# PaulMullowney/hypre

Hardware: AMD Instinct MI355X
Metric: BoomerAMG V-cycle DOF/s (256^3 7-pt Laplacian per GPU, l1-Jacobi V(1,1), fp64) (higher is better)
Workload: dtype f64; 1 GPU; 256x256x256 7-pt Laplacian, 1 rank(s) 1x1x1, PMIS + ext+i(4) + l1-Jacobi V(1,1); transport=none, replicated_from_level=-1, coarse_tail_graph_from_level=-1, coarse_tail_graph_nodes=0, one_workgroup_tail_from_level=6, levels=9

## Files before the change

### hypre_amd/binding.py

```python
import ctypes as C
import os

import numpy as np

HERE = os.path.dirname(os.path.abspath(__file__))
LIB_PATH = os.environ.get("HYPRE_AMD_LIB") or os.path.join(HERE, "lib", "libhypre_amd.so")

HYPRE_MEMORY_HOST = 0
HYPRE_MEMORY_DEVICE = 1

Int = C.c_int
BigInt = C.c_longlong
Real = C.c_double
IntP = C.POINTER(C.c_int)
BigIntP = C.POINTER(C.c_longlong)
RealP = C.POINTER(C.c_double)


class HypreAmdError(RuntimeError):
    pass


class CSRMatrix(C.Structure):
    _fields_ = [("i", IntP), ("j", IntP), ("big_j", BigIntP), ("num_rows", Int), ("num_cols", Int),
# ... 153 lines not shown
    "hypre_CSRMatrixMatvecT": (Int, [Real, CSRp, Vecp, Real, Vecp]),
    "hypre_CSRMatrixMatvecDevice": (Int, [Int, Real, CSRp, Vecp, Real, Vecp, Vecp, Int]),
    "hypre_CSRMatrixSpMVDevice": (Int, [Int, Real, CSRp, Vecp, Real, Vecp, Int]),
    "hypre_amd_CSRMatrixInvalidatePlan": (Int, [CSRp]),
    "hypre_amd_CSRMatrixVerifyPlan": (Int, [CSRp]),
    "hypre_amd_CSRMatrixSetImmutable": (Int, [CSRp, Int]),
    "hypre_amd_CSRMatrixPlanForm": (Int, [CSRp]),
    "hypre_amd_PlanTestFailAlloc": (Int, [Int, Int]),
    "hypre_amd_SetMixedPrecisionValues": (Int, [Int]),
    "hypre_amd_SpmvSetRowSlices": (Int, [Int]),
    "hypre_amd_SpmvSetFusedMultivectors": (Int, [Int]),
    "hypre_amd_SpmvFusedMultivectorLaunches": (Int, []),
    "hypre_amd_CSRMatrixPlanRowSlices": (Int, [CSRp, IntP, IntP]),
    "hypre_amd_CSRMatrixSortRows": (Int, [CSRp, Int]),
    "hypre_amd_SpmvSetBandPolicy": (Int, [Int, Int, Int]),
    "hypre_amd_SpmvSetVariant": (Int, [Int, Int]),
    "hypre_amd_CSRMatrixPlanInfo": (Int, [CSRp, IntP, IntP]),
    "hypre_amd_CSRMatrixPlanStaging": (Int, [CSRp, IntP, RealP]),
    "hypre_amd_SpmvSetValueCodes": (Int, [Int]),
    "hypre_amd_SpmvSetSliceForm": (Int, [Int]),
    "hypre_amd_CSRMatrixPlanSliceForm": (Int, [CSRp]),
    "hypre_amd_SpmvSetSliceClasses": (Int, [Int]),
    "hypre_amd_CSRMatrixPlanSliceClasses": (Int, [CSRp]),
    "hypre_amd_CSRMatrixPlanSliceClassHistogram": (Int, [CSRp, C.POINTER(Int), C.POINTER(Int), C.POINTER(BigInt)]),
    "hypre_amd_CSRMatrixPlanValueCodes": (Int, [CSRp]),
    "hypre_SeqVectorSetConstantValues": (Int, [Vecp, Real]),
    "hypre_SeqVectorCopy": (Int, [Vecp, Vecp]),
    "hypre_SeqVectorScale": (Int, [Real, Vecp]),
    "hypre_SeqVectorAxpy": (Int, [Real, Vecp, Vecp]),
    "hypre_SeqVectorAxpyz": (Int, [Real, Vecp, Real, Vecp, Vecp]),
    "hypre_SeqVectorInnerProd": (Real, [Vecp, Vecp]),
    "hypre_SeqVectorElmdivpy": (Int, [Vecp, Vecp, Vecp]),
    "hypre_SeqVectorElmdivpyMarked": (Int, [Vecp, Vecp, Vecp, IntP, Int]),
    "hypre_SeqVectorSetConstantValuesDevice": (Int, [Vecp, Real]),
    "hypre_SeqVectorScaleDevice": (Int, [Real, Vecp]),
    "hypre_SeqVectorAxpyDevice": (Int, [Real, Vecp, Vecp]),
    "hypre_SeqVectorAxpyzDevice": (Int, [Real, Vecp, Real, Vecp, Vecp]),
    "hypre_SeqVectorInnerProdDevice": (Real, [Vecp, Vecp]),
    "hypre_SeqVectorElmdivpyDevice": (Int, [Vecp, Vecp, Vecp, IntP, Int]),
    "hypreDevice_IVAXPY": (Int, [Int, RealP, RealP, RealP]),
    "hypreDevice_IVAXPYMarked": (Int, [Int, RealP, RealP, RealP, IntP, Int]),
    "hypreDevice_DiagScaleVector2": (Int, [Int, Int, RealP, RealP, Real, RealP, RealP, Int]),
    "hypre_ParCSRMatrixCreate": (ParCSRp, [Int, BigInt, BigInt, BigIntP, BigIntP, Int, Int, Int]),
    "hypre_ParCSRMatrixInitialize_v2": (Int, [ParCSRp, Int]),
    "hypre_ParCSRMatrixDestroy": (Int, [ParCSRp]),
    "hypre_ParCSRMatrixMigrate": (Int, [ParCSRp, Int]),
# ... 230 lines not shown
```

### hypre_amd/csrc/internal.hpp

```cpp
#pragma once

#include <hip/hip_runtime.h>
#include <cstdio>
#include <cstdlib>
#include <cstring>
#include <cstdint>
#include <vector>

#include "HYPRE_amd_utilities.h"
#include "hypre_amd_seq_mv.h"
#include "hypre_amd_comm.h"
#include "hypre_amd_parcsr_mv.h"

#define HIP_CHECK(call)                                                          \
   do {                                                                          \
      hipError_t e_ = (call);                                                    \
      if (e_ != hipSuccess) {                                                    \
         char msg_[512];                                                         \
         snprintf(msg_, sizeof(msg_), "HIP error %d (%s) in %s", (int) e_,       \
                  hipGetErrorString(e_), #call);                                 \
         hypre_error_handler(__FILE__, __LINE__, HYPRE_ERROR_GENERIC, msg_);     \
      }                                                                          \
   } while (0)

// ... 131 lines not shown
void watch_release(MatrixWatch &w);
int *take_stale_slot(int **device_view);
void give_stale_slot(int *slot);
void launch_matrix_fingerprint(const int *Ai, const int *Aj, const double *Aa, int n, int nnz, unsigned long long *fp, int *stale,
                               int record, hipStream_t s);
unsigned long long plan_generation();
bool plan_is_stale(const hypre_CSRMatrix *A);
void launch_build_fp(const HYPRE_Int *Aj, int nnz, int num_tiles, int *fp, hipStream_t s);
SpmvPlan *get_plan(hypre_CSRMatrix *A);
hypre_CSRMatrix *strict_lower_of(hypre_CSRMatrix *A);
void      drop_plan(hypre_CSRMatrix *A);
const float *fp32_values_of(hypre_CSRMatrix *A);
void      set_strict_lower(hypre_CSRMatrix *A, hypre_CSRMatrix *L);

enum SpmvOp
{
   OP_AXPBY   = 0,
   OP_JACOBI  = 1,
   OP_JACOBI_CF = 2,
   OP_TSGS    = 3,
   OP_JACOBI_MAP = 4,
   OP_AXPBY_DIV = 5,
   OP_RESID_RD = 6,
   OP_TSGS_FIRST = 7
};

struct SpmvArgs
{
   const HYPRE_Int     *Ai;
   const HYPRE_Int     *Aj;
   const HYPRE_Complex *Aa;
   const float         *Aa32;
   const unsigned char *Ac8;
   const double        *dict;
   int                  ndict;
   int                  dict_rounded;
   const HYPRE_Complex *x;
   const HYPRE_Complex *b;
   HYPRE_Complex       *y;
   HYPRE_Complex       *aux;
   const HYPRE_Complex *d;
   const HYPRE_Int     *marker;
   int                  marker_val;
   HYPRE_Complex        alpha, beta;
   HYPRE_Complex        scale2;
   int                  fill;
   int                  row_offset;
   int                  last_quad;
   int                  x_last;
   int                  reduce_w;
   int                  gather_t;
   int                  xcd_map;
   const int           *tile_perm;
   const int           *tile_fp;
   int                 *stale;
   const int           *rowmap;
   int                  variant;
   int                  use_rs;
   unsigned             rot;
   int                  nnz;
};
void spmv_default_flags(SpmvArgs &a);

void launch_spmv(const SpmvPlan *plan, const SpmvArgs &args, SpmvOp op, hipStream_t s);
bool spmv_with_scaled_quotient(hypre_CSRMatrix *M, const double *x, double *y, double w, const double *d, double *u);
bool launch_spmv_mv(const SpmvPlan *plan, const SpmvArgs &args, int nv, long xstride, long bstride, long ystride, hipStream_t s);
long &spmv_mv_launches();
bool &spmv_fused_multivectors();
void launch_spmv_rownnz(const HYPRE_Int *rownnz, int num_rownnz, const SpmvArgs &args, hipStream_t s);
void launch_spmv_allrows_update(int num_rows, const SpmvArgs &args, hipStream_t s);
bool device_value_codes(const double *Aa, size_t nnz, unsigned char **codes_out, double **dict_out, double **dict32_out, int *ndict_out,
                        hipStream_t s);
bool device_build_slice_form(SpmvPlan *p, const hypre_CSRMatrix *A, hipStream_t s);
bool device_build_row_slices(SpmvPlan *p, const hypre_CSRMatrix *A, hipStream_t s);
int  &spmv_row_slices();
bool &spmv_slice_classes();
bool &spmv_slice_form();
bool &spmv_value_codes();
void launch_build_tiles(const HYPRE_Int *Ai, int num_rows, int nnz, int num_tiles, int *d_tile_row,
                        int *d_tile_k, hipStream_t s);
void launch_build_xs(const HYPRE_Int *Aj, const int *d_tile_k, int num_tiles, int *xs_cnt, int *xs_desc, unsigned short *lidx,
                     hipStream_t s);
constexpr int SPMV_XS_SEGS = 48;
constexpr int SPMV_XS_CAP  = 4096;
int  device_max_row_nnz(const HYPRE_Int *Ai, int num_rows, hipStream_t s);
void sample_row_bands(const HYPRE_Int *Ai, const HYPRE_Int *Aj, int num_rows, int nsamples, int *host_out, hipStream_t s);

void launch_set(double *y, double v, size_t n, hipStream_t s);
// ... 95 lines not shown
```

### hypre_amd/csrc/par_solve.cpp

```cpp
#include "amg_internal.hpp"
#include <algorithm>
#include <cmath>
#include <string>

using namespace hamd;

namespace hamd {

void AmgPrivate::drop_graph()
{
   if (graph_exec) { (void) hipGraphExecDestroy(graph_exec); graph_exec = nullptr; }
   if (graph) { (void) hipGraphDestroy(graph); graph = nullptr; }
   graph_state = 0; graph_sig = 0; graph_launches = 0;
   graph_cur.clear();
}

void AmgPrivate::release_device()
{
   drop_graph();
   graph_level = -1;
   for (double *p : u_alt) { if (p) { hypre_Free(p, HYPRE_MEMORY_DEVICE); } }
   u_alt.clear(); u_alt_len.clear();
   for (double *p : diag_buf) { if (p) { hypre_Free(p, HYPRE_MEMORY_DEVICE); } }
   diag_buf.clear(); diag_len.clear();
// ... 524 lines not shown
   mix((unsigned long long) d->num_levels); mix((unsigned long long) gl);
   for (int k = 0; k < 4; k++) { mix((unsigned long long) d->grid_relax_type[k]); mix((unsigned long long) d->num_grid_sweeps[k]); }
   mix((unsigned long long) d->relax_order); mix((unsigned long long) d->cycle_type); mix((unsigned long long) d->fcycle);
   mix((unsigned long long) d->user_relax_type); mix((unsigned long long) (d->grid_relax_points != nullptr));
   mix((unsigned long long) pv->mixed_precision); mix((unsigned long long) pv->emulated_threads);
   mix((unsigned long long) (uintptr_t) d->Vtemp->local_vector->data);
   for (int l = gl; l < d->num_levels; l++)
   {
      mixd(d->relax_weight[l]); mixd(d->omega[l]);
      mix((unsigned long long) (uintptr_t) d->A_array[l]->diag->data); mix((unsigned long long) (uintptr_t) d->A_array[l]->diag->j);
      mix((unsigned long long) d->A_array[l]->diag->num_nonzeros);
      if (l < d->num_levels - 1 && d->P_array[l])
      {
         mix((unsigned long long) (uintptr_t) d->P_array[l]->diag->data);
         mix((unsigned long long) (uintptr_t) (d->P_array[l]->diagT ? d->P_array[l]->diagT->data : nullptr));
      }
      mix((unsigned long long) (uintptr_t) F[l]->local_vector->data); mix((unsigned long long) (uintptr_t) U[l]->local_vector->data);
      mix((unsigned long long) (uintptr_t) (d->l1_norms[l] ? d->l1_norms[l]->data : nullptr));
      mix((unsigned long long) (uintptr_t) (l < (int) pv->u_alt.size() ? pv->u_alt[(size_t) l] : nullptr));
      mix((unsigned long long) (uintptr_t) (l < (int) pv->diag_buf.size() ? pv->diag_buf[(size_t) l] : nullptr));
   }
   mix(plan_generation());
   mix((unsigned long long) cycle_fusion());
   mix((unsigned long long) (small_tail_on() ? pv->small_tail_nnz : 0)); mix((unsigned long long) (small_tail_forced_form() + 1));
   mix((unsigned long long) hypre_amd_SetMcLookAhead(-1));
   SpmvArgs a{};
   spmv_default_flags(a);
   mix((unsigned long long) a.variant); mix((unsigned long long) a.gather_t); mix((unsigned long long) a.xcd_map);
   return h;
}

bool is_jacobi_type(int t) { return t == 0 || t == 7 || t == 18; }
bool is_ge_type(int t) { return t == 9 || t == 19 || t == 98 || t == 99 || t == 198 || t == 199; }

}

HYPRE_Int hypre_amd_SetCycleFusion(HYPRE_Int on)
{
   if (on >= 0) { cycle_fusion() = on != 0; }
   return cycle_fusion();
}

HYPRE_Int hypre_amd_SetSmallTail(HYPRE_Int on)
{
   if (on >= 0) { small_tail_on() = on != 0; }
   return small_tail_on();
// ... 180 lines not shown
      arrived_down = false;
      int num_sweep, relax_type;
      if (L > 1) { num_sweep = d->num_grid_sweeps[cycle_param]; relax_type = d->grid_relax_type[cycle_param]; }
      else
      {
         num_sweep = d->num_grid_sweeps[0];
         relax_type = d->user_relax_type;
         if (relax_type == -1) { relax_type = 6; }
      }
      const int *cf = d->CF_marker_array[level] ? d->CF_marker_array[level]->data : nullptr;
      const double *l1 = d->l1_norms[level] ? d->l1_norms[level]->data : nullptr;
      const double *fd = F_array[level]->local_vector->data;
      LevelVec &u = lv[(size_t) level];
      const double w = d->relax_weight[level];

      const bool tail_here = pv->tail != nullptr && level == pv->tail_level;
      if (tail_here)
      {
         err = run_replicated_tail(d, pv, fd, u.home, &cycle_op_count);
         u.cur = u.home;
         zeros[(size_t) level] = 0;
         if (err) { break; }
      }
      for (int j = 0; j < ((tail_here || replayed) ? 0 : num_sweep); j++)
      {
         int relax_points = 0, relax_local = d->relax_order;
         if (L == 1 && d->max_levels > 1) { relax_points = 0; relax_local = 0; }
         else if (old_version) { relax_points = d->grid_relax_points[cycle_param][j]; }
         if (old_version && level < L - 1)
         {
            if (relax_points == 1) { cycle_op_count += A[level + 1]->d_num_nonzeros; }
            else if (relax_points == -1) { cycle_op_count += A[level]->d_num_nonzeros - A[level + 1]->d_num_nonzeros; }
         }
         else { cycle_op_count += A[level]->d_num_nonzeros; }
         if (is_ge_type(relax_type))
         {
            hypre_GaussElimSolve(d, level, relax_type);
            u.cur = u.home;
            zeros[(size_t) level] = 0;
         }
         else if (is_jacobi_type(relax_type))
         {
            int pts[2] = {relax_points, 0}, npass = 1;
            if (!old_version && relax_local == 1 && cycle_param < 3)
            {
               npass = 2;
               pts[0] = cycle_param < 2 ? 1 : -1; pts[1] = -pts[0];
            }
            const double *dg = l1;
            if (relax_type == 0 || !dg)
            {
               double *dd = pv->level_diag(level, n);
               launch_diag_first(A[level]->diag->i, A[level]->diag->data, dd, n, s);
               dg = dd;
            }
            for (int pss = 0; pss < npass; pss++)
            {
               if (zeros[(size_t) level] && relax_type != 0)
               {
                  if (presmoothed[(size_t) level]) { presmoothed[(size_t) level] = 0; }
                  else { launch_scaled_div(w, fd, dg, u.cur, pts[pss] ? cf : nullptr, pts[pss], (size_t) n, s); }
               }
               else
               {
                  dev_jacobi_sweep(A[level], fd, cf, pts[pss], w, dg, u.cur, u.other());
                  u.flip();
               }
               zeros[(size_t) level] = 0;
            }
         }
         else if (relax_type == 15)
         {
            if (j == 0)
            {
               if (pv->cg_smoothers.size() < (size_t) L) { pv->cg_smoothers.resize((size_t) L, nullptr); }
               hypre_Vector uv; hypre_ParVector up;
               wrap(&uv, u.cur, n);
               wrap_par(&up, &uv, A[level]->comm, A[level]->global_num_rows);
               up.all_zeros = zeros[(size_t) level];
               HYPRE_Solver &cg = pv->cg_smoothers[(size_t) level];
               if (!cg)
               {
                  HYPRE_ParCSRPCGCreate(A[level]->comm, &cg);
// ... 54 lines not shown
            hypre_ParVectorSetLocalSize(d->Ztemp, n);
            if (old_version) { err = hypre_BoomerAMGRelax(A[level], F_array[level], (HYPRE_Int *) cf, relax_type, relax_points, w, d->omega[level], (HYPRE_Real *) l1, &up, d->Vtemp, d->Ztemp); }
            else { err = hypre_BoomerAMGRelaxIF(A[level], F_array[level], (HYPRE_Int *) cf, relax_type, relax_local, cycle_param, w, d->omega[level], (HYPRE_Real *) l1, &up, d->Vtemp, d->Ztemp); }
            zeros[(size_t) level] = 0;
            if (hypre_error_flag) { err = 1; }
         }
         if (err) { break; }
      }
      if (err) { break; }

      if (!replayed) { --lev_counter[(size_t) level]; }
      if (!replayed && lev_counter[(size_t) level] >= 0 && level != L - 1 && !tail_here)
      {
         arrived_down = true;
         const int fine = level, coarse = level + 1;
         LevelVec &uc = lv[(size_t) coarse];
         uc.cur = uc.home;
         const int nc = A[coarse]->diag->num_rows;
         const int ctype = d->grid_relax_type[coarse == L - 1 ? 3 : 1];
         const bool overwrites_all = (is_jacobi_type(ctype) && ctype != 0 && !(d->relax_order == 1 && coarse != L - 1) &&
                                      !old_version && d->num_grid_sweeps[coarse == L - 1 ? 3 : 1] > 0) || is_ge_type(ctype);
         if (!overwrites_all) { launch_set(uc.cur, 0.0, (size_t) nc, s); }
         zeros[(size_t) coarse] = 1;
         dev_par_matvec(-1.0, A[fine], u.cur, 1.0, fd, vtemp);
         const int fuse_on = cycle_fusion();
         presmoothed[(size_t) coarse] = 0;
         bool restricted = false;
         if (fuse_on && cycle_nprocs == 1 && overwrites_all && is_jacobi_type(ctype) && d->l1_norms[coarse] && d->l1_norms[coarse]->data &&
             P[fine]->diagT && P[fine]->diagT->memory_location == HYPRE_MEMORY_DEVICE && P[fine]->offd->num_cols == 0)
         {
            restricted = spmv_with_scaled_quotient(P[fine]->diagT, vtemp, F_array[coarse]->local_vector->data, d->relax_weight[coarse],
                                                   d->l1_norms[coarse]->data, uc.cur);
            if (restricted) { presmoothed[(size_t) coarse] = 1; F_array[coarse]->all_zeros = 0; }
         }
         if (!restricted) { dev_par_matvecT(1.0, P[fine], vtemp, 0.0, F_array[coarse]->local_vector->data); }
         ++level;
         lev_counter[(size_t) level] = std::max(lev_counter[(size_t) level], (int) d->cycle_type);
         cycle_param = (level == L - 1) ? 3 : 1;
      }
      else if (level != 0)
      {
         if (capturing && level == gl)
         {
            capturing = false;
            hipGraph_t g = nullptr;
            if (hipStreamEndCapture(s, &g) == hipSuccess && g)
            {
// ... 485 lines not shown
```

### hypre_amd/csrc/seq_mv.cpp

```cpp
#include "internal.hpp"
#include <unordered_map>
#include <unordered_set>
#include <omp.h>
#include <algorithm>

using namespace hamd;

namespace hamd {

struct SpmvVariant { int variant; };
static SpmvVariant &spmv_variant()
{
   static SpmvVariant v = {-1};
   if (v.variant < 0)
   {
      const char *e = getenv("HYPRE_AMD_SPMV_VARIANT");
      v.variant = e ? atoi(e) : 2;
   }
   return v;
}

void spmv_default_flags(SpmvArgs &a)
{
   static int gt = -1, xcd = 8;
// ... 349 lines not shown
   auto it = t.find(A);
   if (it == t.end()) { return true; }
   SpmvPlan *p = it->second;
   if (!p->has_checksum) { return true; }
   const bool same_arrays = p->i == A->i && p->j == A->j && p->a == A->data && p->nnz == A->num_nonzeros &&
                            p->num_rows == A->num_rows && p->num_cols == A->num_cols;
   if (same_arrays && device_csr_checksum(A->i, A->j, A->data, A->num_rows, A->num_nonzeros, stream()) == p->checksum) { return true; }
   drop_plan(A);
   return false;
}

bool &spmv_slice_form()
{
   static bool on = [] { const char *e = getenv("HYPRE_AMD_SPMV_SLICE_FORM"); return !(e && atoi(e) == 0); }();
   return on;
}

bool &spmv_slice_classes()
{
   static bool on = [] { const char *e = getenv("HYPRE_AMD_SPMV_SLICE_CLASSES"); return !(e && atoi(e) == 0); }();
   return on;
}

bool &spmv_fused_multivectors()
{
   static bool on = [] { const char *e = getenv("HYPRE_AMD_SPMV_FUSED_MV"); return !(e && atoi(e) == 0); }();
   return on;
}

bool &spmv_value_codes()
{
   static bool on = [] { const char *e = getenv("HYPRE_AMD_SPMV_VALUE_CODES"); return !(e && atoi(e) == 0); }();
   return on;
}

bool plan_is_stale(const hypre_CSRMatrix *A)
{
   auto &t = plan_table();
   auto it = t.find(A);
   return it != t.end() && it->second->h_stale && __atomic_load_n(it->second->h_stale, __ATOMIC_RELAXED) != 0;
}

const float *fp32_values_of(hypre_CSRMatrix *A)
{
   if (!A || A->num_nonzeros <= 0 || !A->data) { return nullptr; }
   SpmvPlan *p = get_plan(A);
// ... 25 lines not shown
   HIP_CHECK(hipStreamSynchronize(s));
   for (int i = 0; i < n; i++) { off[(size_t) i + 1] = off[(size_t) i] + cnt[(size_t) i]; }
   hypre_Free(d_cnt, HYPRE_MEMORY_DEVICE);
   hypre_CSRMatrix *L = hypre_CSRMatrixCreate(n, A->num_cols, off[(size_t) n]);
   hypre_CSRMatrixInitialize_v2(L, 0, HYPRE_MEMORY_DEVICE);
   hypre_TMemcpy(L->i, off.data(), HYPRE_Int, (size_t) n + 1, HYPRE_MEMORY_DEVICE, HYPRE_MEMORY_HOST);
   if (off[(size_t) n] > 0) { launch_fill_lower(A->i, A->j, A->data, L->i, L->j, L->data, n, s); }
   if (plan->owned) { mark_owned(L); }
   plan->Lstrict = L;
   return L;
}

bool spmv_with_scaled_quotient(hypre_CSRMatrix *M, const double *x, double *y, double w, const double *d, double *u)
{
   if (!M || M->num_rows <= 0 || M->num_nonzeros <= 0 || !d || !u || M->memory_location != HYPRE_MEMORY_DEVICE) { return false; }
   SpmvArgs a{};
   a.Ai = M->i; a.Aj = M->j; a.Aa = M->data; a.Aa32 = nullptr;
   a.x = x; a.b = nullptr; a.y = y; a.d = d; a.aux = u; a.marker = nullptr; a.marker_val = 0;
   a.alpha = 1.0; a.beta = 0.0; a.scale2 = w; a.fill = HYPRE_SPMV_FILL_WHOLE; a.row_offset = 0;
   spmv_default_flags(a);
   launch_spmv(get_plan(M), a, OP_AXPBY_DIV, stream());
   return true;
}
}

extern "C" HYPRE_Int hypre_amd_SpmvSetBandPolicy(HYPRE_Int enabled, HYPRE_Int min_tiles, HYPRE_Int force)
{
   hamd::BandPolicy &bp = hamd::band_policy();
   if (enabled >= 0) { bp.enabled = enabled; }
   if (min_tiles >= 0) { bp.min_tiles = min_tiles; }
   if (force >= 0) { bp.force = force; }
   return hypre_error_flag;
}

extern "C" HYPRE_Int hypre_amd_SpmvSetVariant(HYPRE_Int variant, HYPRE_Int unused)
{
   (void) unused;
   hamd::SpmvVariant &v = hamd::spmv_variant();
   if (variant >= 0) { v.variant = variant; }
   return hypre_error_flag;
}

extern "C" HYPRE_Int hypre_amd_SpmvSetValueCodes(HYPRE_Int on)
{
   if (on >= 0) { hamd::spmv_value_codes() = on != 0; }
   return hypre_error_flag;
// ... 778 lines not shown
```

### hypre_amd/csrc/spmv_kernels.hip

```cpp
#include "amg_internal.hpp"

namespace hamd {

typedef int    v4i __attribute__((ext_vector_type(4)));
typedef int    v2i __attribute__((ext_vector_type(2)));
typedef double v2d __attribute__((ext_vector_type(2)));
typedef float  v4f __attribute__((ext_vector_type(4)));

__device__ __forceinline__ double wave_sum64(double v)
{
#pragma unroll
   for (int off = 32; off > 0; off >>= 1) { v += __shfl_xor(v, off, 64); }
   return v;
}

template <int W>
__device__ __forceinline__ double subwave_sum(double v)
{
#pragma unroll
   for (int off = W / 2; off > 0; off >>= 1) { v += __shfl_xor(v, off, 64); }
   return v;
}

__device__ __forceinline__ bool fill_keep(int fill, int row, int col)
// ... 4 lines not shown
      case HYPRE_SPMV_FILL_LOWER:        return col <= row;
      case HYPRE_SPMV_FILL_UPPER:        return col >= row;
      case HYPRE_SPMV_FILL_STRICT_UPPER: return col >  row;
      default:                           return true;
   }
}

struct RowOps
{
   double b, d, x;
   int    m;
   int    g;
};

template <int OP>
__device__ __forceinline__ RowOps load_row_ops(const SpmvArgs &p, int row)
{
   RowOps o;
   o.b = 0.0; o.d = 1.0; o.x = 0.0; o.m = 0;
   if (OP == OP_JACOBI_MAP) { row = p.rowmap[row]; }
   o.g = row;
   if (OP == OP_AXPBY) { if (p.beta != 0.0) { o.b = p.b[row]; } }
   else if (OP == OP_AXPBY_DIV || OP == OP_RESID_RD) { if (p.beta != 0.0) { o.b = p.b[row]; } o.d = p.d[row]; }
   else if (OP == OP_TSGS_FIRST) { o.d = p.d[row]; o.b = p.x[row]; if (p.beta != 0.0) { o.x = p.aux[row]; } }
   else if (OP == OP_TSGS) { o.d = p.d[row]; o.x = p.aux[row]; }
   else
   {
      o.b = p.b[row]; o.d = p.d[row]; o.x = p.x[row];
      if (OP == OP_JACOBI_CF) { o.m = p.marker[row]; }
      if (OP == OP_JACOBI_MAP) { o.m = p.marker ? p.marker[row] : p.marker_val; }
   }
   return o;
}

template <int OP>
__device__ __forceinline__ void row_epilogue(const SpmvArgs &p, int, double sum, const RowOps &o)
{
   const int row = o.g;
   if (OP == OP_AXPBY || OP == OP_AXPBY_DIV)
   {
      double r = __dmul_rn(p.alpha, sum);
      if (p.beta != 0.0) { r = __fma_rn(p.beta, o.b, r); }
      p.y[row] = r;
      if (OP == OP_AXPBY_DIV) { p.aux[row] = __dmul_rn(p.scale2, r) / o.d; }
   }
   else if (OP == OP_RESID_RD)
   {
      double r = __dmul_rn(p.alpha, sum);
      if (p.beta != 0.0) { r = __fma_rn(p.beta, o.b, r); }
      p.y[row] = __dmul_rn(r, 1.0 / o.d);
   }
   else if (OP == OP_TSGS_FIRST)
   {
      const double z = __dmul_rn(sum, 1.0 / o.d);
      p.y[row] = z;
      p.aux[row] = __fma_rn(p.alpha, z, __dadd_rn(o.x, o.b));
   }
   else if (OP == OP_TSGS)
   {
      const double z = __dmul_rn(sum, 1.0 / o.d);
      p.y[row] = z;
      p.aux[row] = __fma_rn(p.alpha, z, o.x);
   }
   else
   {
      if ((OP == OP_JACOBI_CF || OP == OP_JACOBI_MAP) && o.m != p.marker_val) { p.y[row] = o.x; return; }
      const double t = __fma_rn(p.alpha, o.b, -__dmul_rn(p.alpha, sum));
// ... 1160 lines not shown

   int block = (int) blockIdx.x;
   if (sl_perm)
   {
      if (block >= blocks) { return; }
      block = sl_perm[block];
   }
   else { const int g = block >> 3, c = block & 7; block = (g >> 3) * 64 + c * 8 + (g & 7); }
   if ((unsigned) block >= (unsigned) blocks) { return; }

   const int tid = threadIdx.x, lane = tid & 63;
   const int wave = __builtin_amdgcn_readfirstlane(tid >> 6);
   constexpr int R = SPMV_THREADS / W;
   const int r = block * R + tid / W, sub = tid % W;
   SlLane<CLS, KP> me;
   sl_lane_load<CLS, W, KP>(me, st, p.Ai, block, wave, lane, tid, r, num_rows);
   const RowOps ops = load_row_ops<OP>(p, max(min(r, num_rows - 1), 0));
   const int *dsc = sl_desc + (size_t) block * XS_DESC + XS_WSEG * wave;
   int seg_start[XS_WSEG], seg_ol[XS_WSEG];
#pragma unroll
   for (int j = 0; j < XS_WSEG; j++) { seg_start[j] = dsc[j]; seg_ol[j] = dsc[XS_SEGS + j]; }
   const int k0 = sl_k0[block], k1b = sl_k0[block + 1], fp_plan = sl_fp[block];
   asm volatile("" :: "s"(sl_desc), "s"(sl_k0), "s"(sl_fp), "s"(CLS ? (const void *) st.toff : (const void *) st.data), "s"(st.tab), "s"(p.Ai) : "memory");
#pragma unroll
   for (int j = 0; j < XS_WSEG; j++)
   {
      const unsigned offb = (unsigned) seg_ol[j] >> 16, lanes = (unsigned) seg_ol[j] & 0xffffu;
      if ((unsigned) lane < lanes)
      {
         __builtin_amdgcn_global_load_lds((const __attribute__((address_space(1))) void *) (p.x + (size_t) (unsigned) seg_start[j] + 2 * lane),
                                          (__attribute__((address_space(3))) void *) (reinterpret_cast<char *>(xs) + offb), 16, 0, 0);
      }
   }
   sl_lane_stage<CLS, KP>(me, st, wave, lane, tabl);
   {
      const int dl = (p.ndict + 1) >> 1;
      if (lane < dl - 64 * wave)
      {
         __builtin_amdgcn_global_load_lds((const __attribute__((address_space(1))) void *) (p.dict + 128 * wave + 2 * lane),
                                          (__attribute__((address_space(3))) void *) (reinterpret_cast<char *>(const_cast<double *>(dictl)) + 1024 * wave), 16, 0, 0);
      }
   }
   const int q0 = min(max(k0, 0), nnz - 1), q1 = min(max(k0, 0) + 1, nnz - 1);
   const int fc0 = p.Aj[q0], fc1 = p.Aj[q1];
   const int ck = min(max(min(k0 + 8 * (int) ((4u * p.rot + (unsigned) wave) & 511u) + (lane & 7), k1b - 1), 0), nnz - 1);
   const double ckv = p.Aa[ck];
   const unsigned ckc = p.Ac8[ck];
   __syncthreads();

   const int mylen = sl_lane_words<CLS, W, KP>(me, tid, tabl);
   double sum = 0.0;
#pragma unroll
   for (int j = 0; j < KP; j++)
   {
      const unsigned code = (me.cw[j >> 2] >> (8 * (j & 3))) & 0xffu;
      const unsigned li = (me.lw[j >> 1] >> (16 * (j & 1))) & 0xffffu;
      {
#pragma clang fp contract(off)
         const double pr = dictl[code] * xs[li];
         if (j < mylen) { sum = sum + pr; }
      }
   }
   if (W == 2) { sum += __shfl_xor(sum, 1, 64); }
// ... 1092 lines not shown
      a.dict = rounded ? plan->d_dict32 : plan->d_dict;
      a.dict_rounded = rounded ? 1 : 0;
   }
   a.use_rs = takes_rs(plan, a) ? 1 : 0;
   if (a.use_rs && (handle().fp32_values || a.Aa32))
   {
      SpmvPlan *mp = const_cast<SpmvPlan *>(plan);
      if (!mp->d_rs_val32 && plan_alloc((void **) &mp->d_rs_val32, sizeof(float) * ((size_t) plan->nnz + 64), PLAN_SITE_ROWSLICE))
      {
         launch_f64_to_f32(plan->d_rs_val, mp->d_rs_val32, (size_t) plan->nnz, s);
      }
      if (mp->d_rs_val32) { a.Aa32 = mp->d_rs_val32; } else { a.use_rs = 0; }
   }
   if (handle().fp32_values && !a.Aa32 && !a.Ac8 && plan->nnz > 0)
   {
      SpmvPlan *mp = const_cast<SpmvPlan *>(plan);
      if (!mp->a32)
      {
         HIP_CHECK(hipMalloc((void **) &mp->a32, sizeof(float) * (((size_t) plan->nnz + 3) & ~(size_t) 3)));
         launch_f64_to_f32(plan->a, mp->a32, (size_t) plan->nnz, s);
      }
      a.Aa32 = mp->a32;
   }
   if (a.rowmap && op != OP_JACOBI_MAP) { hypre_error_w_msg(HYPRE_ERROR_ARG, "row map given to an operation that does not read it"); return; }
   {
      const double nz = (double) plan->nnz, nr = (double) plan->num_rows, vw = (a.Aa32 || a.dict_rounded) ? 4.0 : 8.0;
      const double xcols = 8.0 * std::min((double) plan->num_cols, nz);
      double rowb = 0.0;
      switch (op)
      {
         case OP_AXPBY:      rowb = 8.0 + ((a.beta != 0.0) ? 8.0 : 0.0); break;
         case OP_AXPBY_DIV:  rowb = 24.0 + ((a.beta != 0.0) ? 8.0 : 0.0); break;
         case OP_RESID_RD:   rowb = 16.0 + ((a.beta != 0.0) ? 8.0 : 0.0); break;
         case OP_TSGS_FIRST: rowb = 32.0 + ((a.beta != 0.0) ? 8.0 : 0.0); break;
         case OP_JACOBI:     rowb = 24.0; break;
         case OP_JACOBI_CF:  rowb = 28.0; break;
         case OP_JACOBI_MAP: rowb = 28.0 + (a.marker ? 4.0 : 0.0); break;
         case OP_TSGS:       rowb = 32.0; break;
      }
      const double rows_b = 4.0 * (nr + 1.0) + rowb * nr + xcols;
      const bool staged = takes_xs(plan, a);
      const bool slice = staged && a.Ac8 && a.fill == HYPRE_SPMV_FILL_WHOLE && plan->has_slice_form();
      double streamed;
      if (a.use_rs)
      {
         streamed = nz * (vw + 2.0) + (double) plan->rs_blocks * (4.0 * (4 * RS_HDR + SPMV_THREADS + XS_DESC)) + rowb * nr + xcols;
      }
      else if (slice)
      {
         streamed = sl_matrix_bytes(plan, a.ndict) + rowb * nr + xcols;
      }
      else if (staged)
      {
         streamed = nz * ((a.Ac8 ? 1.0 : vw) + 2.0) + rows_b + (double) plan->num_tiles * (4.0 * (XS_DESC + 6) + (a.Ac8 ? 8.0 * a.ndict : 0.0) + ((a.Ac8 || a.Aa32) ? 4.0 * 72.0 : 0.0));
      }
      else { streamed = nz * (vw + 4.0) + rows_b + (plan->tiled ? 8.0 * plan->num_tiles : 0.0); }
      account_bytes(nz * (vw + 4.0) + rows_b, streamed);
   }
   switch (op)
   {
      case OP_AXPBY:     launch_spmv_op<OP_AXPBY>(plan, a, s); break;
      case OP_AXPBY_DIV: launch_spmv_op<OP_AXPBY_DIV>(plan, a, s); break;
      case OP_RESID_RD:  launch_spmv_op<OP_RESID_RD>(plan, a, s); break;
      case OP_TSGS_FIRST: launch_spmv_op<OP_TSGS_FIRST>(plan, a, s); break;
      case OP_JACOBI:    launch_spmv_op<OP_JACOBI>(plan, a, s); break;
      case OP_JACOBI_CF: launch_spmv_op<OP_JACOBI_CF>(plan, a, s); break;
      case OP_JACOBI_MAP: launch_spmv_op<OP_JACOBI_MAP>(plan, a, s); break;
      case OP_TSGS:      launch_spmv_op<OP_TSGS>(plan, a, s); break;
   }
}

template <int NV, bool CODED>
static void launch_xs_mv(const SpmvPlan *plan, const SpmvArgs &a, int stage_elems, int win_elems, int rp_cap, size_t lds,
                         long xstride, long bstride, long ystride, hipStream_t s)
{
   static bool raised = false;
   if (!raised)
   {
      (void) hipFuncSetAttribute((const void *) (spmv_xs_mv_kernel<NV, CODED>), hipFuncAttributeMaxDynamicSharedMemorySize, 160 * 1024);
      (void) hipGetLastError();
      raised = true;
   }
   const int unit = a.tile_perm ? 1 : (a.xcd_map > 0 ? 8 * a.xcd_map : 8);
   const int grid = ((plan->num_tiles + unit - 1) / unit) * unit;
   const int threads = (plan->max_tile_rows > SPMV_THREADS && plan->max_tile_rows <= 320) ? 320 :
                       (plan->max_tile_rows > 320 ? MV_THREADS_MAX : SPMV_THREADS);
   hipLaunchKernelGGL((spmv_xs_mv_kernel<NV, CODED>), dim3(grid), dim3(threads), lds, s, a,
                      plan->d_tile_row, plan->d_tile_k, plan->d_xs_cnt, plan->d_xs_desc, plan->d_lidx,
                      plan->num_tiles, stage_elems, win_elems, rp_cap, plan->xs_launch_units, xstride, bstride, ystride);
}

long &spmv_mv_launches() { static long n = 0; return n; }
// ... 157 lines not shown
```

### include/hypre_amd_seq_mv.h

```cpp
#ifndef HYPRE_AMD_SEQ_MV_H
#define HYPRE_AMD_SEQ_MV_H

#include "HYPRE_amd_utilities.h"

#ifdef __cplusplus
extern "C" {
#endif

typedef struct
{
   HYPRE_Int            *i;
   HYPRE_Int            *j;
   HYPRE_BigInt         *big_j;
   HYPRE_Int             num_rows;
   HYPRE_Int             num_cols;
   HYPRE_Int             num_nonzeros;
   hypre_int            *i_short;
   hypre_int            *j_short;
   HYPRE_Int             owns_data;
   HYPRE_Int             pattern_only;
   HYPRE_Complex        *data;
   HYPRE_Int            *rownnz;
   HYPRE_Int             num_rownnz;
   HYPRE_MemoryLocation  memory_location;
// ... 67 lines not shown
HYPRE_Int hypre_CSRMatrixMatvec(HYPRE_Complex alpha, hypre_CSRMatrix *A, hypre_Vector *x,
                                HYPRE_Complex beta, hypre_Vector *y);
HYPRE_Int hypre_CSRMatrixMatvecT(HYPRE_Complex alpha, hypre_CSRMatrix *A, hypre_Vector *x,
                                 HYPRE_Complex beta, hypre_Vector *y);
HYPRE_Int hypre_CSRMatrixMatvecDevice(HYPRE_Int trans, HYPRE_Complex alpha, hypre_CSRMatrix *A,
                                      hypre_Vector *x, HYPRE_Complex beta, hypre_Vector *b,
                                      hypre_Vector *y, HYPRE_Int offset);
HYPRE_Int hypre_CSRMatrixSpMVDevice(HYPRE_Int trans, HYPRE_Complex alpha, hypre_CSRMatrix *B,
                                    hypre_Vector *x, HYPRE_Complex beta, hypre_Vector *y,
                                    HYPRE_Int fill);

HYPRE_Int hypre_amd_CSRMatrixInvalidatePlan(hypre_CSRMatrix *A);
HYPRE_Int hypre_amd_CSRMatrixVerifyPlan(hypre_CSRMatrix *A);
HYPRE_Int hypre_amd_CSRMatrixSetImmutable(hypre_CSRMatrix *A, HYPRE_Int on);
HYPRE_Int hypre_amd_SetMixedPrecisionValues(HYPRE_Int on);
HYPRE_Int hypre_amd_CSRMatrixPlanForm(hypre_CSRMatrix *A);
HYPRE_Int hypre_amd_PlanTestFailAlloc(HYPRE_Int site, HYPRE_Int nth);
HYPRE_Int hypre_amd_CSRMatrixSortRows(hypre_CSRMatrix *A, HYPRE_Int keep_first);
HYPRE_Int hypre_amd_SpmvSetBandPolicy(HYPRE_Int enabled, HYPRE_Int min_tiles, HYPRE_Int force);
HYPRE_Int hypre_amd_SpmvSetVariant(HYPRE_Int variant, HYPRE_Int unused);
HYPRE_Int hypre_amd_SpmvSetValueCodes(HYPRE_Int on);
HYPRE_Int hypre_amd_SpmvSetSliceForm(HYPRE_Int on);
HYPRE_Int hypre_amd_SpmvSetSliceClasses(HYPRE_Int on);
HYPRE_Int hypre_amd_SpmvSetRowSlices(HYPRE_Int mode);
HYPRE_Int hypre_amd_SpmvSetFusedMultivectors(HYPRE_Int on);
HYPRE_Int hypre_amd_SpmvFusedMultivectorLaunches(void);
HYPRE_Int hypre_amd_CSRMatrixPlanRowSlices(hypre_CSRMatrix *A, HYPRE_Int *rows_per_block, HYPRE_Int *entries_per_lane);
HYPRE_Int hypre_amd_CSRMatrixPlanSliceForm(hypre_CSRMatrix *A);
HYPRE_Int hypre_amd_CSRMatrixPlanSliceClasses(hypre_CSRMatrix *A);
HYPRE_Int hypre_amd_CSRMatrixPlanSliceClassHistogram(hypre_CSRMatrix *A, HYPRE_Int *hist, HYPRE_Int *blocks, HYPRE_BigInt *total);
HYPRE_Int hypre_amd_CSRMatrixPlanValueCodes(hypre_CSRMatrix *A);
HYPRE_Int hypre_amd_CSRMatrixPlanStaging(hypre_CSRMatrix *A, HYPRE_Int *num_tiles, HYPRE_Real *mean_pieces);
HYPRE_Int hypre_amd_CSRMatrixPlanInfo(hypre_CSRMatrix *A, HYPRE_Int *num_tiles, HYPRE_Int *band);

HYPRE_Int hypre_SeqVectorSetConstantValues(hypre_Vector *v, HYPRE_Complex value);
HYPRE_Int hypre_SeqVectorCopy(hypre_Vector *x, hypre_Vector *y);
HYPRE_Int hypre_SeqVectorScale(HYPRE_Complex alpha, hypre_Vector *y);
HYPRE_Int hypre_SeqVectorAxpy(HYPRE_Complex alpha, hypre_Vector *x, hypre_Vector *y);
HYPRE_Int hypre_SeqVectorAxpyz(HYPRE_Complex alpha, hypre_Vector *x, HYPRE_Complex beta,
                               hypre_Vector *y, hypre_Vector *z);
HYPRE_Real hypre_SeqVectorInnerProd(hypre_Vector *x, hypre_Vector *y);
HYPRE_Int hypre_SeqVectorElmdivpy(hypre_Vector *x, hypre_Vector *b, hypre_Vector *y);
HYPRE_Int hypre_SeqVectorElmdivpyMarked(hypre_Vector *x, hypre_Vector *b, hypre_Vector *y,
                                        HYPRE_Int *marker, HYPRE_Int marker_val);
HYPRE_Int hypre_SeqVectorSetConstantValuesDevice(hypre_Vector *v, HYPRE_Complex value);
HYPRE_Int hypre_SeqVectorScaleDevice(HYPRE_Complex alpha, hypre_Vector *y);
// ... 18 lines not shown
```

Measured before the change: 9.026 billion DOF/s.

## Fuse zero-guess presmoothing into the residual SpMV on the down leg

When a level starts from a zero guess with a single l1-Jacobi presweep, the separate scaled-divide kernel that writes u = w*f/d is skipped. Instead a new slice-form SpMV op computes u on the fly in LDS from f and d while staging x, and in the same pass writes both u and the residual f - A*u. This removes one full kernel launch plus one read and write of the vector per descending level, at the cost of a new kernel variant, extra divides during staging, and a fallback path when the plan lacks a slice form.

```diff
diff --git a/hypre_amd/binding.py b/hypre_amd/binding.py
--- a/hypre_amd/binding.py
+++ b/hypre_amd/binding.py
@@ -199,6 +199,9 @@
     "hypre_amd_CSRMatrixPlanSliceForm": (Int, [CSRp]),
     "hypre_amd_SpmvSetSliceClasses": (Int, [Int]),
     "hypre_amd_CSRMatrixPlanSliceClasses": (Int, [CSRp]),
+    "hypre_amd_SetZeroGuessResidual": (Int, [Int]),
+    "hypre_amd_ZeroGuessResidualLaunches": (Int, []),
+    "hypre_amd_CSRMatrixResidualFromZeroGuess": (Int, [CSRp, Real, Vecp, Vecp, Vecp, Vecp]),
     "hypre_amd_CSRMatrixPlanSliceClassHistogram": (Int, [CSRp, C.POINTER(Int), C.POINTER(Int), C.POINTER(BigInt)]),
     "hypre_amd_CSRMatrixPlanValueCodes": (Int, [CSRp]),
     "hypre_SeqVectorSetConstantValues": (Int, [Vecp, Real]),
diff --git a/hypre_amd/csrc/internal.hpp b/hypre_amd/csrc/internal.hpp
--- a/hypre_amd/csrc/internal.hpp
+++ b/hypre_amd/csrc/internal.hpp
@@ -177,7 +177,8 @@
    OP_JACOBI_MAP = 4,
    OP_AXPBY_DIV = 5,
    OP_RESID_RD = 6,
-   OP_TSGS_FIRST = 7
+   OP_TSGS_FIRST = 7,
+   OP_RESID_ZERO = 8
 };
 
 struct SpmvArgs
@@ -219,6 +220,10 @@
 
 void launch_spmv(const SpmvPlan *plan, const SpmvArgs &args, SpmvOp op, hipStream_t s);
 bool spmv_with_scaled_quotient(hypre_CSRMatrix *M, const double *x, double *y, double w, const double *d, double *u);
+bool residual_from_zero_guess(hypre_CSRMatrix *M, double w, const double *f, const double *d, double *u, double alpha, double beta, double *y);
+bool launch_spmv_zero_guess(const SpmvPlan *plan, const SpmvArgs &args, hipStream_t s);
+long &zero_guess_launches();
+bool &zero_guess_residual();
 bool launch_spmv_mv(const SpmvPlan *plan, const SpmvArgs &args, int nv, long xstride, long bstride, long ystride, hipStream_t s);
 long &spmv_mv_launches();
 bool &spmv_fused_multivectors();
diff --git a/hypre_amd/csrc/par_solve.cpp b/hypre_amd/csrc/par_solve.cpp
--- a/hypre_amd/csrc/par_solve.cpp
+++ b/hypre_amd/csrc/par_solve.cpp
@@ -570,6 +570,7 @@
    }
    mix(plan_generation());
    mix((unsigned long long) cycle_fusion());
+   mix((unsigned long long) zero_guess_residual());
    mix((unsigned long long) (small_tail_on() ? pv->small_tail_nnz : 0)); mix((unsigned long long) (small_tail_forced_form() + 1));
    mix((unsigned long long) hypre_amd_SetMcLookAhead(-1));
    SpmvArgs a{};
@@ -796,6 +797,7 @@
          zeros[(size_t) level] = 0;
          if (err) { break; }
       }
+      const double *zero_guess_d = nullptr;
       for (int j = 0; j < ((tail_here || replayed) ? 0 : num_sweep); j++)
       {
          int relax_points = 0, relax_local = d->relax_order;
@@ -832,7 +834,10 @@
             {
                if (zeros[(size_t) level] && relax_type != 0)
                {
+                  const bool descends = lev_counter[(size_t) level] - 1 >= 0 && level != L - 1;
                   if (presmoothed[(size_t) level]) { presmoothed[(size_t) level] = 0; }
+                  else if (cycle_fusion() && zero_guess_residual() && cycle_nprocs == 1 && A[level]->offd->num_cols == 0 && npass == 1 &&
+                           pts[pss] == 0 && num_sweep == 1 && descends && !(st >= 0 && level >= st)) { zero_guess_d = dg; }
                   else { launch_scaled_div(w, fd, dg, u.cur, pts[pss] ? cf : nullptr, pts[pss], (size_t) n, s); }
                }
                else
@@ -933,7 +938,13 @@
                                       !old_version && d->num_grid_sweeps[coarse == L - 1 ? 3 : 1] > 0) || is_ge_type(ctype);
          if (!overwrites_all) { launch_set(uc.cur, 0.0, (size_t) nc, s); }
          zeros[(size_t) coarse] = 1;
-         dev_par_matvec(-1.0, A[fine], u.cur, 1.0, fd, vtemp);
+         bool resid_done = false;
+         if (zero_guess_d)
+         {
+            resid_done = residual_from_zero_guess(A[fine]->diag, w, fd, zero_guess_d, u.cur, -1.0, 1.0, vtemp);
+            if (!resid_done) { launch_scaled_div(w, fd, zero_guess_d, u.cur, nullptr, 0, (size_t) n, s); }
+         }
+         if (!resid_done) { dev_par_matvec(-1.0, A[fine], u.cur, 1.0, fd, vtemp); }
          const int fuse_on = cycle_fusion();
          presmoothed[(size_t) coarse] = 0;
          bool restricted = false;
diff --git a/hypre_amd/csrc/seq_mv.cpp b/hypre_amd/csrc/seq_mv.cpp
--- a/hypre_amd/csrc/seq_mv.cpp
+++ b/hypre_amd/csrc/seq_mv.cpp
@@ -395,6 +395,15 @@
    return on;
 }
 
+}
+extern "C" HYPRE_Int hypre_amd_SetCycleFusion(HYPRE_Int on);
+namespace hamd {
+bool &zero_guess_residual()
+{
+   static bool on = [] { const char *e = getenv("HYPRE_AMD_ZERO_GUESS_RESIDUAL"); return !(e && atoi(e) == 0); }();
+   return on;
+}
+
 bool &spmv_fused_multivectors()
 {
    static bool on = [] { const char *e = getenv("HYPRE_AMD_SPMV_FUSED_MV"); return !(e && atoi(e) == 0); }();
@@ -466,6 +475,49 @@
    launch_spmv(get_plan(M), a, OP_AXPBY_DIV, stream());
    return true;
 }
+
+bool residual_from_zero_guess(hypre_CSRMatrix *M, double w, const double *f, const double *d, double *u, double alpha, double beta, double *y)
+{
+   if (!zero_guess_residual() || !hypre_amd_SetCycleFusion(-1)) { return false; }
+   if (!M || M->num_rows <= 0 || M->num_nonzeros <= 0 || !f || !d || !u || !y || M->memory_location != HYPRE_MEMORY_DEVICE) { return false; }
+   if (M->rownnz && (double) M->num_rownnz < 0.7 * (double) M->num_rows) { return false; }
+   if (plan_is_stale(M)) { return false; }
+   SpmvArgs a{};
+   a.Ai = M->i; a.Aj = M->j; a.Aa = M->data; a.Aa32 = nullptr;
+   a.x = nullptr; a.b = f; a.y = y; a.d = d; a.aux = u; a.marker = nullptr; a.marker_val = 0;
+   a.alpha = alpha; a.beta = beta; a.scale2 = w; a.fill = HYPRE_SPMV_FILL_WHOLE; a.row_offset = 0;
+   spmv_default_flags(a);
+   return launch_spmv_zero_guess(get_plan(M), a, stream());
+}
+}
+
+extern "C" HYPRE_Int hypre_amd_SetZeroGuessResidual(HYPRE_Int on)
+{
+   if (on >= 0) { hamd::zero_guess_residual() = on != 0; }
+   return hamd::zero_guess_residual() ? 1 : 0;
+}
+extern "C" HYPRE_Int hypre_amd_ZeroGuessResidualLaunches(void) { return (HYPRE_Int) hamd::zero_guess_launches(); }
+extern "C" HYPRE_Int hypre_amd_CSRMatrixResidualFromZeroGuess(hypre_CSRMatrix *A, HYPRE_Complex w, hypre_Vector *f, hypre_Vector *d,
+                                                              hypre_Vector *u, hypre_Vector *r)
+{
+   using namespace hamd;
+   if (!A || !f || !d || !u || !r || A->memory_location != HYPRE_MEMORY_DEVICE || f->memory_location != HYPRE_MEMORY_DEVICE ||
+       d->memory_location != HYPRE_MEMORY_DEVICE || u->memory_location != HYPRE_MEMORY_DEVICE || r->memory_location != HYPRE_MEMORY_DEVICE ||
+       f->size < A->num_rows || d->size < A->num_rows || u->size < A->num_rows || r->size < A->num_rows)
+   {
+      hypre_error_w_msg(HYPRE_ERROR_ARG, "hypre_amd_CSRMatrixResidualFromZeroGuess: device matrix and four device vectors of its size");
+      return 0;
+   }
+   (void) get_plan(A);
+   if (!residual_from_zero_guess(A, w, f->data, d->data, u->data, -1.0, 1.0, r->data)) { return 0; }
+   HIP_CHECK(hipStreamSynchronize(stream()));
+   if (plan_is_stale(A))
+   {
+      (void) get_plan(A);
+      if (!residual_from_zero_guess(A, w, f->data, d->data, u->data, -1.0, 1.0, r->data)) { return 0; }
+      HIP_CHECK(hipStreamSynchronize(stream()));
+   }
+   return 1;
 }
 
 extern "C" HYPRE_Int hypre_amd_SpmvSetBandPolicy(HYPRE_Int enabled, HYPRE_Int min_tiles, HYPRE_Int force)
diff --git a/hypre_amd/csrc/spmv_kernels.hip b/hypre_amd/csrc/spmv_kernels.hip
--- a/hypre_amd/csrc/spmv_kernels.hip
+++ b/hypre_amd/csrc/spmv_kernels.hip
@@ -50,6 +50,7 @@
    o.g = row;
    if (OP == OP_AXPBY) { if (p.beta != 0.0) { o.b = p.b[row]; } }
    else if (OP == OP_AXPBY_DIV || OP == OP_RESID_RD) { if (p.beta != 0.0) { o.b = p.b[row]; } o.d = p.d[row]; }
+   else if (OP == OP_RESID_ZERO) { o.b = p.b[row]; o.d = p.d[row]; }
    else if (OP == OP_TSGS_FIRST) { o.d = p.d[row]; o.b = p.x[row]; if (p.beta != 0.0) { o.x = p.aux[row]; } }
    else if (OP == OP_TSGS) { o.d = p.d[row]; o.x = p.aux[row]; }
    else
@@ -71,6 +72,13 @@
       if (p.beta != 0.0) { r = __fma_rn(p.beta, o.b, r); }
       p.y[row] = r;
       if (OP == OP_AXPBY_DIV) { p.aux[row] = __dmul_rn(p.scale2, r) / o.d; }
+   }
+   else if (OP == OP_RESID_ZERO)
+   {
+      double r = __dmul_rn(p.alpha, sum);
+      if (p.beta != 0.0) { r = __fma_rn(p.beta, o.b, r); }
+      p.y[row] = r;
+      p.aux[row] = __dmul_rn(p.scale2, o.b) / o.d;
    }
    else if (OP == OP_RESID_RD)
    {
@@ -1277,14 +1285,17 @@
    for (int j = 0; j < XS_WSEG; j++) { seg_start[j] = dsc[j]; seg_ol[j] = dsc[XS_SEGS + j]; }
    const int k0 = sl_k0[block], k1b = sl_k0[block + 1], fp_plan = sl_fp[block];
    asm volatile("" :: "s"(sl_desc), "s"(sl_k0), "s"(sl_fp), "s"(CLS ? (const void *) st.toff : (const void *) st.data), "s"(st.tab), "s"(p.Ai) : "memory");
-#pragma unroll
-   for (int j = 0; j < XS_WSEG; j++)
-   {
-      const unsigned offb = (unsigned) seg_ol[j] >> 16, lanes = (unsigned) seg_ol[j] & 0xffffu;
-      if ((unsigned) lane < lanes)
-      {
-         __builtin_amdgcn_global_load_lds((const __attribute__((address_space(1))) void *) (p.x + (size_t) (unsigned) seg_start[j] + 2 * lane),
-                                          (__attribute__((address_space(3))) void *) (reinterpret_cast<char *>(xs) + offb), 16, 0, 0);
+   if constexpr (OP != OP_RESID_ZERO)
+   {
+#pragma unroll
+      for (int j = 0; j < XS_WSEG; j++)
+      {
+         const unsigned offb = (unsigned) seg_ol[j] >> 16, lanes = (unsigned) seg_ol[j] & 0xffffu;
+         if ((unsigned) lane < lanes)
+         {
+            __builtin_amdgcn_global_load_lds((const __attribute__((address_space(1))) void *) (p.x + (size_t) (unsigned) seg_start[j] + 2 * lane),
+                                             (__attribute__((address_space(3))) void *) (reinterpret_cast<char *>(xs) + offb), 16, 0, 0);
+         }
       }
    }
    sl_lane_stage<CLS, KP>(me, st, wave, lane, tabl);
@@ -1294,6 +1305,37 @@
       {
          __builtin_amdgcn_global_load_lds((const __attribute__((address_space(1))) void *) (p.dict + 128 * wave + 2 * lane),
                                           (__attribute__((address_space(3))) void *) (reinterpret_cast<char *>(const_cast<double *>(dictl)) + 1024 * wave), 16, 0, 0);
+      }
+   }
+   if constexpr (OP == OP_RESID_ZERO)
+   {
+      constexpr int SL_ZB = 3;
+      static_assert(XS_WSEG % SL_ZB == 0, "whole batches");
+#pragma unroll
+      for (int j0 = 0; j0 < XS_WSEG; j0 += SL_ZB)
+      {
+         if (((unsigned) seg_ol[j0] & 0xffffu) == 0u) { break; }
+         v2d fv[SL_ZB], dv[SL_ZB];
+#pragma unroll
+         for (int jj = 0; jj < SL_ZB; jj++)
+         {
+            fv[jj] = v2d{0.0, 0.0}; dv[jj] = v2d{1.0, 1.0};
+            if ((unsigned) lane < ((unsigned) seg_ol[j0 + jj] & 0xffffu))
+            {
+               fv[jj] = *reinterpret_cast<const v2d *>(p.b + (size_t) (unsigned) seg_start[j0 + jj] + 2 * lane);
+               dv[jj] = *reinterpret_cast<const v2d *>(p.d + (size_t) (unsigned) seg_start[j0 + jj] + 2 * lane);
+            }
+         }
+#pragma unroll
+         for (int jj = 0; jj < SL_ZB; jj++)
+         {
+            const unsigned offb = (unsigned) seg_ol[j0 + jj] >> 16;
+            if ((unsigned) lane < ((unsigned) seg_ol[j0 + jj] & 0xffffu))
+            {
+               const v2d q = {__dmul_rn(p.scale2, fv[jj].x) / dv[jj].x, __dmul_rn(p.scale2, fv[jj].y) / dv[jj].y};
+               *reinterpret_cast<v2d *>(reinterpret_cast<char *>(xs) + offb + 16 * lane) = q;
+            }
+         }
       }
    }
    const int q0 = min(max(k0, 0), nnz - 1), q1 = min(max(k0, 0) + 1, nnz - 1);
@@ -2432,6 +2474,7 @@
       }
       a.Aa32 = mp->a32;
    }
+   if (op == OP_RESID_ZERO) { hypre_error_w_msg(HYPRE_ERROR_ARG, "the residual from a zero guess is launched by launch_spmv_zero_guess"); return; }
    if (a.rowmap && op != OP_JACOBI_MAP) { hypre_error_w_msg(HYPRE_ERROR_ARG, "row map given to an operation that does not read it"); return; }
    {
       const double nz = (double) plan->nnz, nr = (double) plan->num_rows, vw = (a.Aa32 || a.dict_rounded) ? 4.0 : 8.0;
@@ -2447,6 +2490,7 @@
          case OP_JACOBI_CF:  rowb = 28.0; break;
          case OP_JACOBI_MAP: rowb = 28.0 + (a.marker ? 4.0 : 0.0); break;
          case OP_TSGS:       rowb = 32.0; break;
+         case OP_RESID_ZERO: break;
       }
       const double rows_b = 4.0 * (nr + 1.0) + rowb * nr + xcols;
       const bool staged = takes_xs(plan, a);
@@ -2477,7 +2521,39 @@
       case OP_JACOBI_CF: launch_spmv_op<OP_JACOBI_CF>(plan, a, s); break;
       case OP_JACOBI_MAP: launch_spmv_op<OP_JACOBI_MAP>(plan, a, s); break;
       case OP_TSGS:      launch_spmv_op<OP_TSGS>(plan, a, s); break;
-   }
+      case OP_RESID_ZERO: break;
+   }
+}
+
+long &zero_guess_launches() { static long n = 0; return n; }
+bool launch_spmv_zero_guess(const SpmvPlan *plan, const SpmvArgs &args, hipStream_t s)
+{
+   if (plan->num_rows <= 0 || plan->num_rows != plan->num_cols || !plan->has_slice_form() || !plan->d_codes || !args.b || !args.d || !args.aux) { return false; }
+   if (((((uintptr_t) args.b) | ((uintptr_t) args.d) | ((uintptr_t) args.aux)) & 15) != 0 || args.fill != HYPRE_SPMV_FILL_WHOLE) { return false; }
+   SpmvArgs a = args;
+   a.x = args.b;
+   if (!takes_xs(plan, a) || takes_rs(plan, a)) { return false; }
+   a.last_quad = (plan->nnz > 0 ? (int) (plan->nnz - 1) : 0) & ~3;
+   a.x_last = plan->num_cols - 1;
+   a.tile_perm = plan->d_tile_perm;
+   a.tile_fp = plan->d_tile_fp;
+   a.stale = plan->d_stale;
+   a.nnz = plan->nnz;
+   a.rot = const_cast<SpmvPlan *>(plan)->launches++;
+   const bool rounded = handle().fp32_values || a.Aa32 != nullptr;
+   a.Ac8 = plan->d_codes; a.ndict = plan->ndict;
+   a.dict = rounded ? plan->d_dict32 : plan->d_dict;
+   a.dict_rounded = rounded ? 1 : 0;
+   a.use_rs = 0;
+   {
+      const double nz = (double) plan->nnz, nr = (double) plan->num_rows, vw = rounded ? 4.0 : 8.0;
+      const double xcols = 8.0 * std::min((double) plan->num_cols, nz);
+      const double rowb = 8.0 + ((a.beta != 0.0) ? 8.0 : 0.0);
+      account_bytes(24.0 * nr + nz * (vw + 4.0) + 4.0 * (nr + 1.0) + rowb * nr + xcols, sl_matrix_bytes(plan, a.ndict) + 2.0 * xcols + 16.0 * nr);
+   }
+   zero_guess_launches()++;
+   launch_sl<OP_RESID_ZERO>(plan, a, s);
+   return true;
 }
 
 template <int NV, bool CODED>
diff --git a/include/hypre_amd_seq_mv.h b/include/hypre_amd_seq_mv.h
--- a/include/hypre_amd_seq_mv.h
+++ b/include/hypre_amd_seq_mv.h
@@ -113,6 +113,10 @@
 HYPRE_Int hypre_amd_SpmvSetValueCodes(HYPRE_Int on);
 HYPRE_Int hypre_amd_SpmvSetSliceForm(HYPRE_Int on);
 HYPRE_Int hypre_amd_SpmvSetSliceClasses(HYPRE_Int on);
+HYPRE_Int hypre_amd_SetZeroGuessResidual(HYPRE_Int on);
+HYPRE_Int hypre_amd_ZeroGuessResidualLaunches(void);
+HYPRE_Int hypre_amd_CSRMatrixResidualFromZeroGuess(hypre_CSRMatrix *A, HYPRE_Complex w, hypre_Vector *f, hypre_Vector *d,
+                                                   hypre_Vector *u, hypre_Vector *r);
 HYPRE_Int hypre_amd_SpmvSetRowSlices(HYPRE_Int mode);
 HYPRE_Int hypre_amd_SpmvSetFusedMultivectors(HYPRE_Int on);
 HYPRE_Int hypre_amd_SpmvFusedMultivectorLaunches(void);
```

Measured after the change: 9.076 billion DOF/s (median of 6 runs). No clear change (+0.5%).
